# MQinghe/UST-RUN

Hardware: AMD Instinct MI355X
Metric: train images/sec (256x256 U-Net, mixed lb+ulb batch) (higher is better)
Workload: dtype bf16; 1 GPU; fundus 256x256, 2-class U-Net (31.0M params), batch=16+16 per GPU, SSL step = 3 teacher + 5(+1) student forwards, 4 backwards, CE+Dice, SGD+EMA; global_batch=32, parallelism=dp1, fft_mix=device

## Files before the change

### ust-run_amd/csrc/conv_halo_bf16.hip

```cpp
#include "common.h"
#include "loader.h"
#include <stdlib.h>
#include <type_traits>

namespace ustrun {
namespace {

typedef __attribute__((ext_vector_type(8))) elt_t bf16x8;
typedef __attribute__((ext_vector_type(4))) elt_t bf16x4;
typedef __attribute__((address_space(1))) const void gptr_t;
typedef __attribute__((address_space(3))) void lptr_t;


__device__ __attribute__((aligned(16))) const unsigned g_zero16[4] = {0u, 0u, 0u, 0u};

template <int V> using ic = std::integral_constant<int, V>;
template <class T> struct more_value { static constexpr bool value = true; };
template <bool B> struct more_value<std::integral_constant<bool, B>> { static constexpr bool value = B; };

template <int TH, int TW, int BN, int BK, int MI, bool POOL, int NT, bool XF, int DIL = 1, bool BREG = false, bool M16 = false, bool BNS = false,
          int LINW = 0>
__global__ __launch_bounds__(256, (TH * TW * BN >= 512 * 64 && BN == 64 ? 1 : 2)) void conv3x3_halo_bf16_kernel(const IgemmArgs a, const int tiles_x, const int tiles_y,
                                                                   const int nt_total) {
    static_assert(BK == 32, "80-byte patch rows hold one 32-channel chunk");
    constexpr bool LIN = LINW > 0;
    constexpr int RP = LINW + 1;
    constexpr int TM = TH * TW;
    static_assert(!LIN || (DIL == 1 && !POOL && TW == 32 && BREG && RP > 8), "linear tiles: un-dilated, un-pooled, 32-position sub-tiles");
    static_assert(!M16 || (BREG && !XF), "the 16x16x32 build: plain sources, weights through registers");
    static_assert(!BNS || M16, "BatchNorm-backward sums ride on the 16x16x32 epilogue (8 channels of a pixel per lane)");
    static_assert(!BREG || NT <= 2, "register-fed weights: 16 registers per tap and set");
    constexpr int HW2 = LIN ? RP : TW + 2 * DIL;
    constexpr int SR = 32 / TW;
    constexpr int WM = TH / (SR * MI), WN = 4 / WM;
    static_assert(WM * WN == 4 && BN == WN * 64, "4 waves, 64 channels per wave");
    constexpr int HP = LIN ? TM + 2 * RP + 2 : (TH + 2 * DIL) * HW2;
    constexpr int PITCH = 80;
    constexpr int DSLOTS = (HP * 5 + 63) / 64 * 64;
    constexpr int XSLOTS = (HP * 4 + 63) / 64 * 64;
    constexpr int AIT = (DSLOTS + 255) / 256;
    constexpr int NSTG = (9 + NT - 1) / NT;
    constexpr int BATCH = (AIT + NSTG - 2) / (NSTG - 1);
    static_assert(BATCH * (NSTG - 1) >= AIT, "staging fits the chunk");
    constexpr int NP = POOL ? 4 : 1;
    constexpr int ABYTES = (BREG ? AIT * 256 : DSLOTS) * 16;
    constexpr int BCH = (BK / 8) * BN;
    constexpr int BIT = BCH / 256;
    static_assert(BCH % 256 == 0, "B tile must be a whole number of wave-instructions per wave");
    constexpr int RAWB = XF ? BATCH * NP * 4096 : 0;
    constexpr int BBYTES = BREG ? 0 : 2 * NT * BCH * 16;
    constexpr bool SKEW = XF && 2 * ABYTES + BBYTES + 2 * RAWB + 512 <= 81920;
    constexpr int NRAW = SKEW ? 2 : 1;

    extern __shared__ __attribute__((aligned(16))) char smem[];
    char* As = smem;
    char* Bs = smem + 2 * ABYTES;
    char* Raw = Bs + BBYTES;
    char* Cst = Raw + NRAW * RAWB;

    const int IS = LIN ? (a.Ho + 1) * RP : 1;
    const int lin_full = LIN ? a.N / tiles_y : 0;
    const int mt_total = LIN ? lin_full * tiles_x + ((a.N - lin_full * tiles_y) * IS + TM - 1) / TM : a.N * tiles_y * tiles_x;
    const int ntiles = mt_total * nt_total;
    int bid = blockIdx.x;
    {
        const int q = ntiles / 8, r = ntiles % 8, xcd = bid % 8, j = bid / 8;
        bid = (xcd < r ? xcd * (q + 1) : r * (q + 1) + (xcd - r) * q) + j;
    }
    const int mtile = bid / nt_total, ntile = bid % nt_total;
    const int n0 = ntile * BN;
    const int lpass = LIN ? min(mtile / tiles_x, lin_full) : 0;
    const int img = LIN ? lpass * tiles_y : mtile / (tiles_y * tiles_x);
    const int nimg = LIN ? min(tiles_y, a.N - img) : 1;
    const int P0 = LIN ? (mtile - lpass * tiles_x) * TM : 0;
    const int trem = LIN ? 0 : mtile - img * tiles_y * tiles_x;
    const int y0 = LIN ? 0 : (trem / tiles_x) * TH, x0 = LIN ? 0 : (trem % tiles_x) * TW;

    const int tid = threadIdx.x, lane = tid & 63;
    const int wave = __builtin_amdgcn_readfirstlane(tid >> 6);
    const int wm = wave / WN, wn = wave % WN;
    const int l31 = lane & 31, lh = lane >> 5;

    const int nchunk = a.Cin / BK;
    const int K8 = a.Cin / 8;
    const elt_t* Wp = (const elt_t*)a.W;
    const elt_t* zsrc = (const elt_t*)g_zero16;
    const bool wflip = a.dstep < 0;

    constexpr int OOB = (int)0x80000000;
    int aoff[AIT];
    unsigned aokm = 0;
    __amdgpu_buffer_rsrc_t ars = __builtin_amdgcn_make_buffer_rsrc((void*)g_zero16, 0, 0, 0x00020000);
    int asoff = 0;
    int cur_src = -1;
    float a_floor = 0.f;
    const elt_t* aptr = nullptr;
    long dq1 = 0, dq2 = 0;
    f32x4 asc0, asc1, ash0, ash1;
    const int p8 = tid & 3;
    auto src_setup = [&](const SrcDev& S) {
        a_floor = S.relu ? 0.f : -__builtin_inff();
        dq1 = S.sW; dq2 = S.sH;
        const int by = y0 - DIL - S.off_y, bx = x0 - DIL - S.off_x;
        aokm = 0;
        int tq = tid;
        asm volatile("" : "+v"(tq));
#pragma unroll
        for (int i = 0; i < AIT; ++i) {
            const int q = tq + 256 * i;
            const int hp = XF ? (q >> 2) : q / 5;
            const int g = XF ? (tq & 3) : q - 5 * hp;
            if constexpr (LIN) {
                const int F = P0 - RP - 1 + hp, Fc = F < 0 ? 0 : F;
                const int il = Fc / IS, rem = Fc - il * IS, r = rem / RP, c = rem - r * RP;
                const int ly = r - S.off_y, lx = c - S.off_x;
                const bool ok = hp < HP && g < 4 && F >= 0 && il < nimg && r < a.Ho && c < LINW && ly >= 0 && ly < S.LH && lx >= 0 && lx < S.LW;
                aoff[i] = ok ? 2 * ((int)((long)il * S.sN + (long)ly * S.sH + (long)lx * S.sW) + 8 * g) : OOB;
                aokm |= (ok ? 1u : 0u) << i;
                continue;
            }
            const int hy = hp / HW2, hx = hp - hy * HW2;
            const int ly = by + hy, lx = bx + hx;
            const bool ok = hp < HP && g < 4 && ly >= 0 && ly < S.LH && lx >= 0 && lx < S.LW;
            aoff[i] = ok ? 2 * ((int)((POOL ? 2 : 1) * ((long)ly * S.sH + (long)lx * S.sW)) + 8 * g) : OOB;
            aokm |= (ok ? 1u : 0u) << i;
        }
        ars = __builtin_amdgcn_make_buffer_rsrc((void*)((const char*)S.ptr + (long)img * S.sN * 2), 0, 0x7fffffff, 0x00020000);
    };
    auto stage_begin = [&](int c, bool from_lds = true) {
        const int cg = c * BK;
        const int second = (a.nsrc == 2 && cg >= a.src[0].C) ? 1 : 0;
        const SrcDev S = pick_src(a.src[0], a.src[1], second != 0);
        const int cl = cg - (second ? a.src[0].C : 0);
        if (second != cur_src) { src_setup(S); cur_src = second; }
        aptr = (const elt_t*)S.ptr + (img * S.sN + cl);
        asoff = 2 * cl;
        asc0 = asc1 = (f32x4){1.f, 1.f, 1.f, 1.f}; ash0 = ash1 = (f32x4){0.f, 0.f, 0.f, 0.f};
        if (S.scale && !from_lds) {
            const long goff = S.gN > 0 ? (long)(img / S.gN) * S.gstride : 0;
            const float* sc = S.scale + goff + cl + 8 * p8;
            const float* sh = S.shift + goff + cl + 8 * p8;
            asc0 = *(const f32x4*)sc; asc1 = *(const f32x4*)(sc + 4);
            ash0 = *(const f32x4*)sh; ash1 = *(const f32x4*)(sh + 4);
        } else if (S.scale) {
            const char* cs = Cst + (c & 1) * 256 + p8 * 32;
            asc0 = *(const f32x4*)cs; asc1 = *(const f32x4*)(cs + 16);
            ash0 = *(const f32x4*)(cs + 128); ash1 = *(const f32x4*)(cs + 144);
        }
    };
    auto dma_consts = [&](int c) {
        const int cg = c * BK;
        const bool second = (a.nsrc == 2 && cg >= a.src[0].C);
        const SrcDev S = pick_src(a.src[0], a.src[1], second);
        const int cl = cg - (second ? a.src[0].C : 0);
        if (S.scale && wave == 0 && lane < 16) {
            const long goff = S.gN > 0 ? (long)(img / S.gN) * S.gstride : 0;
            const float* src = (lane < 8 ? S.scale : S.shift) + goff + cl + 4 * (lane & 7);
            __builtin_amdgcn_global_load_lds((gptr_t*)src, (lptr_t*)(Cst + (c & 1) * 256), 16, 0, 0);
        }
// ... 4 lines not shown
        if constexpr (XF) {
#pragma unroll
            for (int q = 0; q < NP; ++q) {
                const int d = 2 * (int)((q & 1 ? dq1 : 0) + (q & 2 ? dq2 : 0));
                dma16_buf_s(vo, ars, asoff + d, raw + ((b * NP + q) * 256 + wave * 64) * 16);
            }
        } else {
            dma16_buf_s(vo, ars, asoff, Adst + (256 * i + wave * 64) * 16);
        }
    };
    auto act8 = [&](bf16x8 r, f32x4& lo, f32x4& hi) {
        lo = (f32x4){(float)r[0], (float)r[1], (float)r[2], (float)r[3]} * asc0 + ash0;
        hi = (f32x4){(float)r[4], (float)r[5], (float)r[6], (float)r[7]} * asc1 + ash1;
#pragma unroll
        for (int q = 0; q < 4; ++q) {
            lo[q] = __builtin_amdgcn_fmed3f(lo[q], a_floor, __builtin_inff());
            hi[q] = __builtin_amdgcn_fmed3f(hi[q], a_floor, __builtin_inff());
        }
    };
    typedef __attribute__((ext_vector_type(4))) unsigned u32x4;
    auto xform8 = [&](const bf16x8* r, bool inimg) {
        f32x4 lo, hi;
        act8(r[0], lo, hi);
#pragma unroll
        for (int q = 1; q < NP; ++q) {
            f32x4 l2, h2;
            act8(r[q], l2, h2);
            lo = max4(lo, l2); hi = max4(hi, h2);
        }
        bf16x8 h;
        h[0] = (elt_t)lo[0]; h[1] = (elt_t)lo[1]; h[2] = (elt_t)lo[2]; h[3] = (elt_t)lo[3];
        h[4] = (elt_t)hi[0]; h[5] = (elt_t)hi[1]; h[6] = (elt_t)hi[2]; h[7] = (elt_t)hi[3];
        u32x4 u = __builtin_bit_cast(u32x4, h);
#pragma unroll
        for (int q = 0; q < 4; ++q) u[q] = inimg ? u[q] : 0u;
        return __builtin_bit_cast(bf16x8, u);
    };
    const int xw0 = (tid >> 2) * PITCH + p8 * 16;
    auto raw_read = [&](int b, const char* raw, bf16x8* r) {
#pragma unroll
        for (int q = 0; q < NP; ++q) r[q] = *(const bf16x8*)(raw + ((b * NP + q) * 256 + tid) * 16);
    };
    auto xform_store = [&](int i, const bf16x8* r, char* Adst, bool live, const char* raw) {
        const bool in_patch = live && (tid >> 2) + 64 * i < HP;
        char* dst = in_patch ? Adst + xw0 + i * 64 * PITCH : (char*)raw + tid * 16;
        *(bf16x8*)dst = xform8(r, (aokm >> i) & 1u);
    };
    const elt_t* wthr[BIT];
#pragma unroll
    for (int i = 0; i < BIT; ++i) {
        const int idx = tid + 256 * i, o = idx / BN, n = idx % BN;
        wthr[i] = Wp + ((long)o * a.Cout + n0 + n) * 8;
    }
    auto dma_B = [&](int c, int tap, int slot) {
        const int wt = wflip ? 8 - tap : tap;
        const long woff = ((long)wt * K8 + c * (BK / 8)) * a.Cout * 8;
        char* dst = Bs + slot * (BCH * 16);
#pragma unroll
        for (int i = 0; i < BIT; ++i)
            __builtin_amdgcn_global_load_lds((gptr_t*)(wthr[i] + woff), (lptr_t*)(dst + (wave * 64 + 256 * i) * 16), 16, 0, 0);
    };

    const __amdgpu_buffer_rsrc_t wrs = __builtin_amdgcn_make_buffer_rsrc((void*)Wp, 0, (int)min((long)9 * K8 * a.Cout * 16, 0x7fffffffL), 0x00020000);
    const int bvoff0 = (lh * a.Cout + n0 + wn * 64 + l31) * 16, bvoff1 = bvoff0 + 2 * a.Cout * 16;
    const int bvoff16 = ((lane >> 4) * a.Cout + n0 + wn * 64 + (lane & 15)) * 16;
    bf16x8 bnx[NT][BK / 16][2];
    auto load_B = [&](int c, int tap, int k) {
        const int wt = wflip ? 8 - tap : tap;
        const int soff = __builtin_amdgcn_readfirstlane((int)(((long)wt * K8 + c * (BK / 8)) * a.Cout * 16));
        if constexpr (M16)
            asm volatile("s_nop 4\n\tbuffer_load_dwordx4 %0, %4, %5, %6 offen\n\tbuffer_load_dwordx4 %1, %4, %5, %6 offen offset:256\n\t"
                         "buffer_load_dwordx4 %2, %4, %5, %6 offen offset:512\n\tbuffer_load_dwordx4 %3, %4, %5, %6 offen offset:768"
                         : "=&v"(bnx[k][0][0]), "=&v"(bnx[k][0][1]), "=&v"(bnx[k][1][0]), "=&v"(bnx[k][1][1])
                         : "v"(bvoff16), "s"(wrs), "s"(soff) : "memory");
        else
        asm volatile("s_nop 4\n\tbuffer_load_dwordx4 %0, %4, %6, %7 offen\n\tbuffer_load_dwordx4 %1, %4, %6, %7 offen offset:512\n\t"
                     "buffer_load_dwordx4 %2, %5, %6, %7 offen\n\tbuffer_load_dwordx4 %3, %5, %6, %7 offen offset:512"
                     : "=&v"(bnx[k][0][0]), "=&v"(bnx[k][0][1]), "=&v"(bnx[k][1][0]), "=&v"(bnx[k][1][1])
                     : "v"(bvoff0), "v"(bvoff1), "s"(wrs), "s"(soff) : "memory");
    };

    f32x16 acc[M16 ? 1 : MI][2];
    f32x4 acc16[M16 ? MI : 1][2][4];
#pragma unroll
    for (int i = 0; i < (M16 ? 1 : MI); ++i)
#pragma unroll
        for (int j = 0; j < 2; ++j)
#pragma unroll
            for (int r = 0; r < 16; ++r) acc[i][j][r] = 0.f;
#pragma unroll
    for (int i = 0; i < (M16 ? MI : 1); ++i)
#pragma unroll
        for (int h = 0; h < 2; ++h)
#pragma unroll
            for (int g = 0; g < 4; ++g) acc16[i][h][g] = (f32x4){0.f, 0.f, 0.f, 0.f};

    const int afrag0 = LIN ? (M16 ? (wm * MI * 32 + (lane & 15)) * PITCH + (lane >> 4) * 16 : (wm * MI * 32 + l31) * PITCH + lh * 16)
                     : M16 ? ((wm * SR * MI) * HW2 + (lane & 15)) * PITCH + (lane >> 4) * 16
                           : ((wm * SR * MI + (TW == 16 ? (l31 >> 4) : 0)) * HW2 + (l31 & (TW - 1))) * PITCH + lh * 16;
    const int bfrag0 = (lh * BN + wn * 64 + l31) * 16;
    const int nstage = nchunk * NSTG;

    if constexpr (BREG) {
#pragma unroll
        for (int k = 0; k < NT; ++k) load_B(0, k, k);
    } else {
#pragma unroll
        for (int k = 0; k < NT; ++k) dma_B(0, k, k);
    }
    if (nchunk > 1) dma_consts(1);
    stage_begin(0, false);
    if constexpr (XF) {
        bf16x8 pv[AIT][NP];
#pragma unroll
        for (int i = 0; i < AIT; ++i) {
            const bool ok = (aokm >> i) & 1u;
            const elt_t* src = ok ? (const elt_t*)((const char*)aptr + aoff[i]) : zsrc;
#pragma unroll
            for (int q = 0; q < NP; ++q) pv[i][q] = *(const bf16x8*)(src + (ok ? (q & 1 ? dq1 : 0) + (q & 2 ? dq2 : 0) : 0));
        }
#pragma unroll
        for (int i = 0; i < AIT; ++i)
        {
            const bool in_patch = (tid >> 2) + 64 * i < HP;
            *(bf16x8*)(in_patch ? As + xw0 + i * 64 * PITCH : Raw + tid * 16) = xform8(pv[i], (aokm >> i) & 1u);
        }
    } else {
#pragma unroll
        for (int i = 0; i < AIT; ++i)
            if (wave_has(i)) issue_one(i, 0, As, nullptr);
    }
    asm volatile("s_waitcnt vmcnt(0)" ::: "memory");
    __syncthreads();

    bf16x8 acar[MI];
    constexpr bool PEEL = BREG && !XF;
    constexpr bool CT = BREG && XF && SKEW;
    constexpr bool APIPE = BREG && !XF;
    int ni_prev = 0;
    auto chunk = [&](const int c, auto more_c) __attribute__((always_inline)) {
        const bool more = more_c;
        constexpr bool morec = more_value<decltype(more_c)>::value;
        const char* Afrag = As + (c & 1) * ABYTES + afrag0;
        char* Anext = As + ((c + 1) & 1) * ABYTES;
        if (more) stage_begin(c + 1);
        auto stage = [&](auto ic_j) {
            constexpr int j = decltype(ic_j)::value;
            constexpr int t0 = j * NT, nt = (9 - t0 < NT) ? 9 - t0 : NT;
            constexpr int jn = (j + 1) % NSTG, tn0 = jn * NT, nn = (9 - tn0 < NT) ? 9 - tn0 : NT;
            const int s = c * NSTG + j;
            bf16x8 bcur[NT][BK / 16][2];
            const bool has_next = PEEL ? (morec || j < NSTG - 1) : (CT || s + 1 < nstage);
            const int nb_new = (BREG && has_next) ? 4 * nn : 0;
            if constexpr (BREG) {
#pragma unroll
                for (int k = 0; k < NT; ++k)
#pragma unroll
                    for (int ks = 0; ks < BK / 16; ++ks) { bcur[k][ks][0] = bnx[k][ks][0]; bcur[k][ks][1] = bnx[k][ks][1]; }
                if (has_next) {
#pragma unroll
                    for (int k = 0; k < nn; ++k) load_B(jn == 0 ? (CT && !more ? c : c + 1) : c, tn0 + k, k);
                }
            } else if (s + 1 < nstage) {
#pragma unroll
                for (int k = 0; k < nn; ++k) dma_B(jn == 0 ? c + 1 : c, tn0 + k, ((s + 1) & 1) * NT + k);
            }
            if constexpr (j == NSTG - 1) { if (c + 2 < nchunk) dma_consts(c + 2); }
            char* rawW = Raw + (SKEW ? (s & 1) * RAWB : 0);
            const char* rawR = Raw + (SKEW ? ((s & 1) ^ 1) * RAWB : 0);
            int ni = 0;
            if constexpr (j < NSTG - 1) {
                if (CT || more) {
#pragma unroll
                    for (int b = 0; b < BATCH; ++b) {
                        constexpr int dummy = 0; (void)dummy;
                        if (j * BATCH + b < AIT && wave_has(j * BATCH + b)) { issue_one(j * BATCH + b, b, Anext, rawW, more); ni += NP; }
                    }
                }
            }
            __builtin_amdgcn_sched_barrier(0);
            if constexpr (BREG) {
                if constexpr (PEEL || CT) {
                    constexpr auto pieces = [](int jj) constexpr {
                        int n = 0;
                        if ((CT || morec) && jj >= 0 && jj < NSTG - 1)
                            for (int b = 0; b < BATCH; ++b) n += (jj * BATCH + b < AIT) ? NP : 0;
                        return n;
                    };
                    constexpr int younger = ((CT || morec || j < NSTG - 1) ? 4 * nn : 0) + pieces(j) + (XF ? 0 : pieces(j - 1));
                    static_assert(younger < 64, "vmcnt is a 6-bit counter");
                    asm volatile("s_waitcnt vmcnt(%0)" :: "n"(younger) : "memory");
                } else {
                    const int younger = nb_new + ni + (XF ? 0 : ni_prev);
                    switch (younger < 12 ? younger : 12) {
                        case 12: asm volatile("s_waitcnt vmcnt(12)" ::: "memory"); break;
                        case 11: asm volatile("s_waitcnt vmcnt(11)" ::: "memory"); break;
                        case 10: asm volatile("s_waitcnt vmcnt(10)" ::: "memory"); break;
                        case 9: asm volatile("s_waitcnt vmcnt(9)" ::: "memory"); break;
                        case 8: asm volatile("s_waitcnt vmcnt(8)" ::: "memory"); break;
                        case 7: asm volatile("s_waitcnt vmcnt(7)" ::: "memory"); break;
                        case 6: asm volatile("s_waitcnt vmcnt(6)" ::: "memory"); break;
                        case 5: asm volatile("s_waitcnt vmcnt(5)" ::: "memory"); break;
                        case 4: asm volatile("s_waitcnt vmcnt(4)" ::: "memory"); break;
                        case 3: asm volatile("s_waitcnt vmcnt(3)" ::: "memory"); break;
                        case 2: asm volatile("s_waitcnt vmcnt(2)" ::: "memory"); break;
                        case 1: asm volatile("s_waitcnt vmcnt(1)" ::: "memory"); break;
                        default: asm volatile("s_waitcnt vmcnt(0)" ::: "memory"); break;
                    }
                    ni_prev = ni;
                }
#pragma unroll
                for (int k = 0; k < NT; ++k)
#pragma unroll
                    for (int ks = 0; ks < BK / 16; ++ks) asm volatile("" : "+v"(bcur[k][ks][0]), "+v"(bcur[k][ks][1]));
                __builtin_amdgcn_sched_barrier(0);
            }
            auto afrag = [&](int tap, int ks, int i) __attribute__((always_inline)) {
                if constexpr (LIN)
                    return *(const bf16x8*)(Afrag + (32 * i + (M16 ? 16 * ks : 0) + (tap / 3) * RP + tap % 3) * PITCH + (M16 ? 0 : ks * 32));
                else if constexpr (M16)
                    return *(const bf16x8*)(Afrag + ((DIL * (tap / 3) + SR * i + (TW == 16 ? ks : 0)) * HW2 + DIL * (tap % 3) + (TW == 16 ? 0 : 16 * ks)) * PITCH);
                else
                return *(const bf16x8*)(Afrag + ((DIL * (tap / 3) + SR * i) * HW2 + DIL * (tap % 3)) * PITCH + ks * 32);
            };
            if constexpr (APIPE) {
                if constexpr (j == 0) {
#pragma unroll
// ... 89 lines not shown
                            for (int g = 0; g < 4; ++g)
                                acc16[i][ks][g] = USTRUN_MFMA_16x16x32(bf[k][g >> 1][g & 1], af[k][ks][i], acc16[i][ks][g], 0, 0, 0);
                        } else {
                        acc[i][0] = USTRUN_MFMA_32x32x16(af[k][ks][i], bf[k][ks][0], acc[i][0], 0, 0, 0);
                        acc[i][1] = USTRUN_MFMA_32x32x16(af[k][ks][i], bf[k][ks][1], acc[i][1], 0, 0, 0);
                        }
                    }
            }
            if constexpr (SKEW) {
#pragma unroll
                for (int b = 0; b < nitem; ++b) xform_store(jx * BATCH + b, rr[b], Anext, more, rawR);
            }
            constexpr int nmfma = nt * (BK / 16) * MI * (M16 ? 4 : 2);
            constexpr int vpm = !SKEW ? 0 : (nitem * (NP * 26 + 14) + nmfma - 1) / nmfma;
            if constexpr (APIPE) {
                if constexpr ((j == 0 ? MI : 0) + nitem * NP > 0) __builtin_amdgcn_sched_group_barrier(0x100, (j == 0 ? MI : 0) + nitem * NP, 0);
                if constexpr (M16) {
#pragma unroll
                    for (int h = 0; h < nt * (BK / 16); ++h) {
                        const bool next_read = h + 1 < nt * (BK / 16) || j < NSTG - 1;
#pragma unroll
                        for (int i = 0; i < MI; ++i) {
                            __builtin_amdgcn_sched_group_barrier(0x008, 4, 0);
                            if (next_read) __builtin_amdgcn_sched_group_barrier(0x100, 1, 0);
                        }
                    }
                } else
#pragma unroll
                for (int h = 0; h < nt * (BK / 16); ++h) {
                    const bool next_read = h + 1 < nt * (BK / 16) || j < NSTG - 1;
#pragma unroll
                    for (int m = 0; m < (M16 ? 4 : 2) * MI; ++m) {
                        if (m == 2 && next_read) __builtin_amdgcn_sched_group_barrier(0x100, MI, 0);
                        __builtin_amdgcn_sched_group_barrier(0x008, 1, 0);
                        if constexpr (vpm > 0) __builtin_amdgcn_sched_group_barrier(0x002, vpm, 0);
                    }
                }
                if constexpr (nitem > 0) __builtin_amdgcn_sched_group_barrier(0x200, nitem, 0);
            } else if constexpr (SKEW) {
                constexpr int nread = nt * (BK / 16) * ((BREG ? 0 : 2) + MI) + nitem * NP;
                __builtin_amdgcn_sched_group_barrier(0x100, nread, 0);
#pragma unroll
                for (int m = 0; m < nmfma; ++m) {
                    __builtin_amdgcn_sched_group_barrier(0x008, 1, 0);
                    if constexpr (vpm > 0) __builtin_amdgcn_sched_group_barrier(0x002, vpm, 0);
                }
                if constexpr (nitem > 0) __builtin_amdgcn_sched_group_barrier(0x200, nitem, 0);
            }
            __builtin_amdgcn_sched_barrier(0);
            if constexpr (BREG && j < NSTG - 1 && (!XF || SKEW)) {
            } else if constexpr (!XF && j < NSTG - 1) {
                if (ni == 0) asm volatile("s_waitcnt vmcnt(0)" ::: "memory");
                else if (ni == 1) asm volatile("s_waitcnt vmcnt(1)" ::: "memory");
                else asm volatile("s_waitcnt vmcnt(2)" ::: "memory");
            } else {
                asm volatile("s_waitcnt vmcnt(0)" ::: "memory");
            }
            if constexpr (!SKEW && nitem > 0) {
                if (more) {
#pragma unroll
                    for (int b = 0; b < nitem; ++b) {
                        if (256 * (jx * BATCH + b) + wave * 64 < XSLOTS) {
                            raw_read(b, rawR, rr[b]);
                            xform_store(jx * BATCH + b, rr[b], Anext, true, rawR);
                        }
                    }
                }
            }
            if constexpr (!BREG || j == NSTG - 1) {
                asm volatile("s_waitcnt lgkmcnt(0)" ::: "memory");
                __builtin_amdgcn_s_barrier();
            }
            asm volatile("" ::: "memory");
        };
        stage(ic<0>{}); stage(ic<1>{}); stage(ic<2>{}); stage(ic<3>{}); stage(ic<4>{});
        if constexpr (NSTG > 5) { stage(ic<5>{}); stage(ic<6>{}); stage(ic<7>{}); stage(ic<8>{}); }
    };
    if constexpr (PEEL) {
        for (int c = 0; c + 1 < nchunk; ++c) chunk(c, std::true_type{});
        chunk(nchunk - 1, std::false_type{});
    } else {
        for (int c = 0; c < nchunk; ++c) chunk(c, c + 1 < nchunk);
    }

    const int C1 = a.Cout - a.C0;
    typedef __attribute__((ext_vector_type(2))) float f32x2;
    typedef __attribute__((ext_vector_type(2))) elt_t bf16x2;
    f32x2 s1v[2] = {{0.f, 0.f}, {0.f, 0.f}}, s2v[2] = {{0.f, 0.f}, {0.f, 0.f}};
    float s1p[8] = {0.f, 0.f, 0.f, 0.f, 0.f, 0.f, 0.f, 0.f}, s2p[8] = {0.f, 0.f, 0.f, 0.f, 0.f, 0.f, 0.f, 0.f};
    auto stat_piece = [&](const bf16x8 v8, bool ok) {
#pragma unroll
        for (int q = 0; q < 8; ++q) {
            const float f = ok ? (float)v8[q] : 0.f;
            s1p[q] += f; s2p[q] += f * f;
        }
    };
    float bsc[8], bsh[8];
    if constexpr (BNS) {
        const long go = a.bn_gN > 0 ? (long)(img / a.bn_gN) * a.bn_gstride : 0;
        const float* ps = a.bnsc + go + n0 + wn * 64 + (lane & 7) * 8;
        const float* pb = a.bnsh + go + n0 + wn * 64 + (lane & 7) * 8;
        const f32x4 s0 = *(const f32x4*)ps, s1_ = *(const f32x4*)(ps + 4), b0 = *(const f32x4*)pb, b1 = *(const f32x4*)(pb + 4);
#pragma unroll
        for (int q = 0; q < 4; ++q) { bsc[q] = s0[q]; bsc[4 + q] = s1_[q]; bsh[q] = b0[q]; bsh[4 + q] = b1[q]; }
    }
    auto bns_piece = [&](const bf16x8 v8, const bf16x8 y8, bool ok) {
#pragma unroll
        for (int q = 0; q < 8; ++q) {
            const float yf = (float)y8[q];
            const float dz = (ok && yf * bsc[q] + bsh[q] > 0.f) ? (float)v8[q] : 0.f;
            s1p[q] += dz; s2p[q] += dz * yf;
        }
    };
    constexpr int EPITCH = 144;
    char* ep = smem + wave * (32 * EPITCH);
    const bool full = !LIN && y0 + TH <= a.Ho && x0 + TW <= a.Wo;
    int e_il = 0, e_r = 0, e_c = 0;
    unsigned vmask = 0xffffffffu;
    auto lin_pos = [&](int P, int& il, int& r, int& c) { il = P / IS; const int rem = P - il * IS; r = rem / RP; c = rem - r * RP; };
    if constexpr (LIN) lin_pos(P0 + wm * MI * 32 + (lane >> 3), e_il, e_r, e_c);
    auto park = [&](int i, auto mask_c, auto stat_c) {
        constexpr bool MASK = decltype(mask_c)::value, STAT = decltype(stat_c)::value;
        const int oyb = y0 + wm * SR * MI + SR * i;
        if constexpr (M16) {
#pragma unroll
            for (int h = 0; h < 2; ++h)
#pragma unroll
                for (int g = 0; g < 4; ++g) {
                    const f32x4 v = acc16[M16 ? i : 0][h][g];
                    bf16x4 h4;
                    h4[0] = (elt_t)v[0]; h4[1] = (elt_t)v[1]; h4[2] = (elt_t)v[2]; h4[3] = (elt_t)v[3];
                    *(bf16x4*)(ep + (16 * h + (lane & 15)) * EPITCH + (16 * g + 4 * (lane >> 4)) * 2) = h4;
                }
        } else {
#pragma unroll
        for (int j = 0; j < 2; ++j) {
#pragma unroll
            for (int r = 0; r < 16; r += 2) {
                const int row = (r & 3) + 8 * (r >> 2) + 4 * lh;
                const f32x2 v = {acc[M16 ? 0 : i][j][r], acc[M16 ? 0 : i][j][r + 1]};
                const bf16x2 h = __builtin_convertvector(v, bf16x2);
                *(elt_t*)(ep + row * EPITCH + (j * 32 + l31) * 2) = h[0];
                *(elt_t*)(ep + (row + 1) * EPITCH + (j * 32 + l31) * 2) = h[1];
                if (!STAT) continue;
                f32x2 f = __builtin_convertvector(h, f32x2);
                if (MASK && LIN) {
                    if (!((vmask >> row) & 1u)) f[0] = 0.f;
                    if (!((vmask >> (row + 1)) & 1u)) f[1] = 0.f;
                } else if (MASK) {
                    const int oy0 = oyb + (TW == 16 ? (row >> 4) : 0), ox0 = x0 + (row & (TW - 1));
                    const int oy1 = oyb + (TW == 16 ? ((row + 1) >> 4) : 0), ox1 = x0 + ((row + 1) & (TW - 1));
                    if (!(oy0 < a.Ho && ox0 < a.Wo)) f[0] = 0.f;
                    if (!(oy1 < a.Ho && ox1 < a.Wo)) f[1] = 0.f;
                }
                s1v[j] += f;
                s2v[j] += f * f;
            }
        }
        }
    };
#pragma unroll
    for (int i = 0; i < MI; ++i) {
        const int oyb = y0 + wm * SR * MI + SR * i;
        if constexpr (LIN && !M16) {
            if (a.stat) {
                int il, r, c;
                lin_pos(P0 + wm * MI * 32 + 32 * i + l31, il, r, c);
                vmask = (unsigned)__builtin_amdgcn_ballot_w64(il < nimg && r < a.Ho && c < LINW);
            }
        }
        if constexpr (M16) park(i, std::false_type{}, std::false_type{});
        else {
        if (!a.stat) park(i, std::false_type{}, std::false_type{});
        else if (full) park(i, std::false_type{}, std::true_type{});
        else park(i, std::true_type{}, std::true_type{});
        }
        __builtin_amdgcn_fence(__ATOMIC_RELEASE, "wavefront");
        __builtin_amdgcn_wave_barrier();
        __builtin_amdgcn_fence(__ATOMIC_ACQUIRE, "wavefront");
        if (full && n0 + wn * 64 + 64 <= a.C0) {
            const int r0 = lane >> 3, ch = lane & 7;
            elt_t* base = (elt_t*)a.out0 + (((long)img * a.Ho + oyb) * a.Wo + x0) * a.C0 + n0 + wn * 64 + ch * 8;
#pragma unroll
            for (int t = 0; t < 4; ++t) {
                const int row = r0 + 8 * t;
                const bf16x8 v8 = *(const bf16x8*)(ep + row * EPITCH + ch * 16);
                const long off = TW == 16 ? ((long)(row >> 4) * a.Wo + (row & 15)) * a.C0 : (long)row * a.C0;
                *(bf16x8*)(base + off) = v8;
                if constexpr (BNS) bns_piece(v8, *(const bf16x8*)((const elt_t*)a.bny + (base - (elt_t*)a.out0) + off), true);
                else if constexpr (M16) { if (a.stat) stat_piece(v8, true); }
            }
        } else
#pragma unroll
        for (int t = 0; t < 4; ++t) {
            const int idx = lane + 64 * t, row = idx >> 3, ch = idx & 7;
            const bf16x8 v8 = *(const bf16x8*)(ep + row * EPITCH + ch * 16);
            const int oy = LIN ? e_r : oyb + (TW == 16 ? (row >> 4) : 0), ox = LIN ? e_c : x0 + (row & (TW - 1));
            const int oimg = LIN ? img + e_il : img;
            const bool inb = LIN ? (e_il < nimg && e_r < a.Ho && e_c < LINW) : (oy < a.Ho && ox < a.Wo);
            if constexpr (LIN) {
                e_c += 8;
                if (e_c >= RP) { e_c -= RP; if (++e_r > a.Ho) { e_r = 0; ++e_il; } }
            }
            const int col = n0 + wn * 64 + ch * 8;
            if constexpr (BNS) {
                const bool ok = inb && col < a.C0;
                const long eo = ok ? (((long)oimg * a.Ho + oy) * a.Wo + ox) * a.C0 + col : 0;
                bns_piece(v8, *(const bf16x8*)((const elt_t*)a.bny + eo), ok);
            } else if constexpr (M16) { if (a.stat) stat_piece(v8, inb); }
            if (inb) {
                if (col < a.C0) {
                    *(bf16x8*)((elt_t*)a.out0 + (((long)oimg * a.Ho + oy) * a.Wo + ox) * a.C0 + col) = v8;
                } else {
                    const int y1 = oy - a.o1y, x1 = ox - a.o1x;
                    if (y1 >= 0 && y1 < a.H1 && x1 >= 0 && x1 < a.W1)
                        *(bf16x8*)((elt_t*)a.out1 + (((long)oimg * a.H1 + y1) * a.W1 + x1) * C1 + (col - a.C0)) = v8;
                }
            }
        }
        __builtin_amdgcn_fence(__ATOMIC_RELEASE, "wavefront");
        __builtin_amdgcn_wave_barrier();
        __builtin_amdgcn_fence(__ATOMIC_ACQUIRE, "wavefront");
    }
    float s1[2] = {s1v[0][0] + s1v[0][1], s1v[1][0] + s1v[1][1]}, s2[2] = {s2v[0][0] + s2v[0][1], s2v[1][0] + s2v[1][1]};
    if (a.stat) {
        float* red = (float*)(smem + 4 * 32 * EPITCH);
        if constexpr (M16) {
#pragma unroll
            for (int q = 0; q < 8; ++q) {
#pragma unroll
                for (int o = 8; o < 64; o <<= 1) { s1p[q] += __shfl_xor(s1p[q], o); s2p[q] += __shfl_xor(s2p[q], o); }
                if (lane < 8) {
                    red[(wm * 2 + 0) * BN + wn * 64 + lane * 8 + q] = s1p[q];
                    red[(wm * 2 + 1) * BN + wn * 64 + lane * 8 + q] = s2p[q];
                }
            }
        } else
#pragma unroll
        for (int j = 0; j < 2; ++j) {
            s1[j] += __shfl_xor(s1[j], 32);
            s2[j] += __shfl_xor(s2[j], 32);
            if (lh == 0) {
                red[(wm * 2 + 0) * BN + wn * 64 + j * 32 + l31] = s1[j];
                red[(wm * 2 + 1) * BN + wn * 64 + j * 32 + l31] = s2[j];
            }
        }
        __syncthreads();
        constexpr int SROWS = TH / 8;
        constexpr int WPS = WM / SROWS;
        for (int t = tid; t < SROWS * 2 * BN; t += 256) {
            const int h = t / (2 * BN), q = (t / BN) % 2, cc = t % BN;
            float v = 0.f;
#pragma unroll
            for (int w = 0; w < WPS; ++w) v += red[((h * WPS + w) * 2 + q) * BN + cc];
            a.stat[((long)(mtile * SROWS + h) * 2 + q) * a.Cout + n0 + cc] = v;
        }
    }
}

thread_local int g_last_variant = 0;

struct LinPlan { int gN, tpp, mtiles, last_rows; };
static LinPlan lin_plan(const IgemmArgs& a) {
    int g = a.pass_gN > 0 ? a.pass_gN : 0;
    for (int i = 0; i < a.nsrc && !g; ++i)
        if (a.src[i].gN > 0) g = a.src[i].gN;
    if (!g && a.bn_gN > 0) g = a.bn_gN;
    if (g <= 0 || g > a.N) g = a.N;
    const long IS = (long)(a.Ho + 1) * (a.Wo + 1);
    const int tpp = (int)cdiv(g * IS, 256L), full = a.N / g, tailN = a.N - full * g, tail = (int)cdiv(tailN * IS, 256L);
    return {g, tpp, full * tpp + tail, tailN ? tail : (full > 1 ? tpp : -1)};
}

template <int TH, int TW, int BN, int BK, int MI, bool POOL, int NT, bool XF, int DIL = 1, bool BREG = false, bool M16 = false, bool BNS = false,
          int LINW = 0>
int launch_xf(const IgemmArgs& a, hipStream_t st) {
    g_last_variant = (LINW ? (1 << 30 | LINW << 16) : (TH << 24 | TW << 16)) | BN << 8 | (M16 ? 0x80 : 0) | MI << 4 | NT << 2 | (POOL ? 2 : 0) | (XF ? 1 : 0);
    const LinPlan lp = LINW ? lin_plan(a) : LinPlan{0, 0, 0, -1};
    const int tx = LINW ? lp.tpp : cdiv(a.Wb, TW), ty = LINW ? lp.gN : cdiv(a.Hb, TH), nt = a.Cout / BN;
    constexpr int DSLOTS = ((LINW ? TH * TW + 2 * (LINW + 1) + 2 : (TH + 2 * DIL) * (TW + 2 * DIL)) * 5 + 63) / 64 * 64;
    constexpr int AIT = (DSLOTS + 255) / 256, NSTG = (9 + NT - 1) / NT, BATCH = (AIT + NSTG - 2) / (NSTG - 1);
    const size_t rawb = XF ? (size_t)BATCH * (POOL ? 4 : 1) * 4096 : 0;
    const size_t fixed = 2 * (size_t)(BREG ? AIT * 256 : DSLOTS) * 16 + (BREG ? 0 : 2 * NT * (size_t)(BK / 8) * BN * 16) + 512;
    const size_t lds = fixed + (XF && fixed + 2 * rawb <= 81920 ? 2 : 1) * rawb;
    dim3 grid((LINW ? lp.mtiles : a.N * ty * tx) * nt), block(256);
    if (lds > 64 * 1024)
        USTRUN_TRY(ensure_dynamic_lds((const void*)conv3x3_halo_bf16_kernel<TH, TW, BN, BK, MI, POOL, NT, XF, DIL, BREG, M16, BNS, LINW>, (int)lds, "conv3x3_halo_bf16"));
    hipLaunchKernelGGL((conv3x3_halo_bf16_kernel<TH, TW, BN, BK, MI, POOL, NT, XF, DIL, BREG, M16, BNS, LINW>), grid, block, lds, st, a, tx, ty, nt);
    USTRUN_LAUNCH_CHECK("conv3x3_halo_bf16");
    return 0;
}

template <int TH, int TW, int BN, int BK, int MI, bool POOL, int NT = 1>
int launch_cfg(const IgemmArgs& a, hipStream_t st) {
    bool xf = POOL;
    for (int i = 0; i < a.nsrc; ++i) xf |= a.src[i].scale != nullptr || a.src[i].relu != 0;
    if constexpr (POOL) return launch_xf<TH, TW, BN, BK, MI, POOL, NT, true>(a, st);
    else {
        {
            {
                const bool m16 = !(g_debug_flags & 8) && !(g_debug_flags & 2097152) && ((g_debug_flags & 32768) || (!xf && MI == 4 && NT == 1));
                if constexpr (MI == 4 && NT == 1 && BN == 128) {
                    if (a.bny) {
                        USTRUN_CHECK(m16 && !xf && a.stat && a.bnsc && a.bnsh, "conv3x3_halo: BatchNorm-backward sums need a plain source on the 16x16x32 build");
                        return launch_xf<TH, TW, BN, BK, MI, POOL, NT, false, 1, true, true, true>(a, st);
                    }
                }
                if (m16 && !xf)
                    return launch_xf<TH, TW, BN, BK, MI, POOL, NT, false, 1, true, true>(a, st);
            }
            if (!(g_debug_flags & 8))
                return xf ? launch_xf<TH, TW, BN, BK, MI, POOL, NT, true, 1, true>(a, st) : launch_xf<TH, TW, BN, BK, MI, POOL, NT, false, 1, true>(a, st);
        }
        return xf ? launch_xf<TH, TW, BN, BK, MI, POOL, NT, true>(a, st) : launch_xf<TH, TW, BN, BK, MI, POOL, NT, false>(a, st);
    }
}

}

int halo_last_variant() { return g_last_variant; }
static int halo_dilation(const IgemmArgs& a) { return a.dstep < 0 ? -a.dstep : a.dstep; }
void set_last_variant(int v) { g_last_variant = v; }

int halo_stat_rows(int N, int H, int W) { return N * cdiv(H, 8) * cdiv(W, 16); }

bool halo_supported(const IgemmArgs& a) {
    if (a.nseg != 9 || a.nz != 1 || a.s_in != 1 || a.s_out != 1 || a.segw != 3) return false;
    const int dil = a.dstep < 0 ? -a.dstep : a.dstep;
    if (a.d0 != -a.dstep || !(dil == 1 || dil == 2 || dil == 4)) return false;
    bool pool = false;
    if (a.out_esz != 2 || (a.C0 & 7) || ((a.Cout - a.C0) & 7) || a.bias) return false;
    for (int i = 0; i < a.nsrc; ++i) {
        if (a.src[i].sC != 1 || (a.src[i].C & 7) || a.src[i].esz != 2) return false;
        pool |= a.src[i].pool != 0;
    }
    const int BK = 32;
    if (a.Cin % BK || a.Cout % 64) return false;
    if (a.nsrc == 2 && (a.src[0].C % BK)) return false;
    if (pool && (a.nsrc != 1 || a.Cout % 128)) return false;
    if (a.Hb < 4 || a.Wb < 8) return false;
    if (dil > 1 && (pool || a.nsrc != 1)) return false;
    return true;
}

int halo_tile128(const IgemmArgs& a);
static double halo_rect_score(const IgemmArgs& a);

int halo_linear_w(const IgemmArgs& a) {
    if ((g_debug_flags2 & 1) || (g_debug_flags & (8 | 2097152 | 32768)) || ((g_debug_flags >> 10) & 3)) return 0;
    if (!halo_supported(a) || halo_dilation(a) != 1 || a.Cout % 128 || a.Hb != a.Ho || a.Wb != a.Wo) return 0;
    const int w = a.Wo;
    if (!(w == 18 || w == 24 || w == 36 || w == 72)) return 0;
    int g = a.pass_gN > 0 ? a.pass_gN : 0;
    for (int i = 0; i < a.nsrc; ++i) {
        if (a.src[i].pool) return 0;
        if (a.src[i].gN > 0) { if (g && g != a.src[i].gN) return 0; g = a.src[i].gN; }
    }
    if (a.bny && a.bn_gN > 0 && g && g != a.bn_gN) return 0;
    const LinPlan lp = lin_plan(a);
    for (int i = 0; i < a.nsrc; ++i)
        if ((long)lp.gN * a.src[i].sN * 2 >= (1L << 31) - 4096) return 0;
    if ((long)lp.mtiles * (a.Cout / 128) < 160) return 0;
    const double lin = (double)a.N * a.Ho * a.Wo / (lp.mtiles * 256.0);
    return lin > 1.05 * halo_rect_score(a) ? w : 0;
}
int halo_linear_last_pass_rows(const IgemmArgs& a) { return halo_linear_w(a) ? lin_plan(a).last_rows : -1; }

bool halo_bnsum_supported(const IgemmArgs& a) {
    if (!halo_supported(a) || a.nsrc != 1 || a.out1 || a.C0 != a.Cout || a.Cout % 128) return false;
    if (a.src[0].scale || a.src[0].relu || a.src[0].pool) return false;
    if ((g_debug_flags & (8 | 2097152))) return false;
// ... 112 lines not shown
```

Baseline: 1161 images/sec.

## Add persistent walking mode to 8x32 halo conv that chains tiles per block

For the plain-source 8x32 M16 halo conv variant, launches a reduced grid (about 512/nt blocks, sized per group) in which each block walks a contiguous run of spatial tiles. The next tile's prologue (weight and patch loads) is issued into the alternate patch buffer before the current tile's epilogue, and the epilogue scratch is moved into the finished buffer. This aims to cut block launch and prologue latency and overlap the next tile's loads with the store epilogue. In exchange it adds more complex buffer-parity bookkeeping and possible load imbalance from the fixed partitioning.

```diff
diff --git a/ust-run_amd/csrc/conv_halo_bf16.hip b/ust-run_amd/csrc/conv_halo_bf16.hip
--- a/ust-run_amd/csrc/conv_halo_bf16.hip
+++ b/ust-run_amd/csrc/conv_halo_bf16.hip
@@ -18,11 +18,13 @@
 template <class T> struct more_value { static constexpr bool value = true; };
 template <bool B> struct more_value<std::integral_constant<bool, B>> { static constexpr bool value = B; };
 
+struct WalkPlan { int g, bfull, btail, run; };
 template <int TH, int TW, int BN, int BK, int MI, bool POOL, int NT, bool XF, int DIL = 1, bool BREG = false, bool M16 = false, bool BNS = false,
-          int LINW = 0>
+          int LINW = 0, bool WALK = false>
 __global__ __launch_bounds__(256, (TH * TW * BN >= 512 * 64 && BN == 64 ? 1 : 2)) void conv3x3_halo_bf16_kernel(const IgemmArgs a, const int tiles_x, const int tiles_y,
-                                                                   const int nt_total) {
+                                                                   const int nt_total, const WalkPlan wp) {
     static_assert(BK == 32, "80-byte patch rows hold one 32-channel chunk");
+    static_assert(!WALK || (LINW == 0 && BREG && !XF && !BNS && !POOL && DIL == 1 && TH == 8 && TW == 32), "walking form: the 8 x 32 tiles, plain sources, register-fed weights");
     constexpr bool LIN = LINW > 0;
     constexpr int RP = LINW + 1;
     constexpr int TM = TH * TW;
@@ -64,17 +66,29 @@
     const int ntiles = mt_total * nt_total;
     int bid = blockIdx.x;
     {
-        const int q = ntiles / 8, r = ntiles % 8, xcd = bid % 8, j = bid / 8;
+        const int nb = WALK ? (int)gridDim.x : ntiles;
+        const int q = nb / 8, r = nb % 8, xcd = bid % 8, j = bid / 8;
         bid = (xcd < r ? xcd * (q + 1) : r * (q + 1) + (xcd - r) * q) + j;
     }
-    const int mtile = bid / nt_total, ntile = bid % nt_total;
+    int mtile = bid / nt_total;
+    const int ntile = bid % nt_total;
+    int tend = 0;
+    if constexpr (WALK) {
+        const int tpi = tiles_y * tiles_x, nfull = a.N / wp.g;
+        const int p = min(mtile / wp.bfull, nfull), pb = mtile - p * wp.bfull;
+        const int T = (p < nfull ? wp.g : a.N - nfull * wp.g) * tpi, B = p < nfull ? wp.bfull : wp.btail;
+        const int f = wp.run ? pb * wp.run : (int)((long)pb * T / B);
+        const int l = wp.run ? min(f + wp.run, T) : (int)((long)(pb + 1) * T / B);
+        mtile = p * wp.g * tpi + f;
+        tend = p * wp.g * tpi + l;
+    }
     const int n0 = ntile * BN;
     const int lpass = LIN ? min(mtile / tiles_x, lin_full) : 0;
-    const int img = LIN ? lpass * tiles_y : mtile / (tiles_y * tiles_x);
+    int img = LIN ? lpass * tiles_y : mtile / (tiles_y * tiles_x);
     const int nimg = LIN ? min(tiles_y, a.N - img) : 1;
     const int P0 = LIN ? (mtile - lpass * tiles_x) * TM : 0;
     const int trem = LIN ? 0 : mtile - img * tiles_y * tiles_x;
-    const int y0 = LIN ? 0 : (trem / tiles_x) * TH, x0 = LIN ? 0 : (trem % tiles_x) * TW;
+    int y0 = LIN ? 0 : (trem / tiles_x) * TH, x0 = LIN ? 0 : (trem % tiles_x) * TW;
 
     const int tid = threadIdx.x, lane = tid & 63;
     const int wave = __builtin_amdgcn_readfirstlane(tid >> 6);
@@ -245,18 +259,21 @@
 
     f32x16 acc[M16 ? 1 : MI][2];
     f32x4 acc16[M16 ? MI : 1][2][4];
-#pragma unroll
-    for (int i = 0; i < (M16 ? 1 : MI); ++i)
-#pragma unroll
-        for (int j = 0; j < 2; ++j)
-#pragma unroll
-            for (int r = 0; r < 16; ++r) acc[i][j][r] = 0.f;
-#pragma unroll
-    for (int i = 0; i < (M16 ? MI : 1); ++i)
-#pragma unroll
-        for (int h = 0; h < 2; ++h)
-#pragma unroll
-            for (int g = 0; g < 4; ++g) acc16[i][h][g] = (f32x4){0.f, 0.f, 0.f, 0.f};
+    auto acc_zero = [&]() {
+#pragma unroll
+        for (int i = 0; i < (M16 ? 1 : MI); ++i)
+#pragma unroll
+            for (int j = 0; j < 2; ++j)
+#pragma unroll
+                for (int r = 0; r < 16; ++r) acc[i][j][r] = 0.f;
+#pragma unroll
+        for (int i = 0; i < (M16 ? MI : 1); ++i)
+#pragma unroll
+            for (int h = 0; h < 2; ++h)
+#pragma unroll
+                for (int g = 0; g < 4; ++g) acc16[i][h][g] = (f32x4){0.f, 0.f, 0.f, 0.f};
+    };
+    if constexpr (!WALK) acc_zero();
 
     const int afrag0 = LIN ? (M16 ? (wm * MI * 32 + (lane & 15)) * PITCH + (lane >> 4) * 16 : (wm * MI * 32 + l31) * PITCH + lh * 16)
                      : M16 ? ((wm * SR * MI) * HW2 + (lane & 15)) * PITCH + (lane >> 4) * 16
@@ -264,37 +281,45 @@
     const int bfrag0 = (lh * BN + wn * 64 + l31) * 16;
     const int nstage = nchunk * NSTG;
 
-    if constexpr (BREG) {
-#pragma unroll
-        for (int k = 0; k < NT; ++k) load_B(0, k, k);
-    } else {
-#pragma unroll
-        for (int k = 0; k < NT; ++k) dma_B(0, k, k);
-    }
-    if (nchunk > 1) dma_consts(1);
-    stage_begin(0, false);
-    if constexpr (XF) {
-        bf16x8 pv[AIT][NP];
-#pragma unroll
-        for (int i = 0; i < AIT; ++i) {
-            const bool ok = (aokm >> i) & 1u;
-            const elt_t* src = ok ? (const elt_t*)((const char*)aptr + aoff[i]) : zsrc;
-#pragma unroll
-            for (int q = 0; q < NP; ++q) pv[i][q] = *(const bf16x8*)(src + (ok ? (q & 1 ? dq1 : 0) + (q & 2 ? dq2 : 0) : 0));
-        }
-#pragma unroll
-        for (int i = 0; i < AIT; ++i)
-        {
-            const bool in_patch = (tid >> 2) + 64 * i < HP;
-            *(bf16x8*)(in_patch ? As + xw0 + i * 64 * PITCH : Raw + tid * 16) = xform8(pv[i], (aokm >> i) & 1u);
-        }
-    } else {
-#pragma unroll
-        for (int i = 0; i < AIT; ++i)
-            if (wave_has(i)) issue_one(i, 0, As, nullptr);
-    }
+    int pbase = 0;
+    auto prologue = [&]() {
+        char* A0 = As + pbase * ABYTES;
+        if constexpr (BREG) {
+#pragma unroll
+            for (int k = 0; k < NT; ++k) load_B(0, k, k);
+        } else {
+#pragma unroll
+            for (int k = 0; k < NT; ++k) dma_B(0, k, k);
+        }
+        if constexpr (!WALK) { if (nchunk > 1) dma_consts(1); }
+        else cur_src = -1;
+        stage_begin(0, false);
+        if constexpr (XF) {
+            bf16x8 pv[AIT][NP];
+#pragma unroll
+            for (int i = 0; i < AIT; ++i) {
+                const bool ok = (aokm >> i) & 1u;
+                const elt_t* src = ok ? (const elt_t*)((const char*)aptr + aoff[i]) : zsrc;
+#pragma unroll
+                for (int q = 0; q < NP; ++q) pv[i][q] = *(const bf16x8*)(src + (ok ? (q & 1 ? dq1 : 0) + (q & 2 ? dq2 : 0) : 0));
+            }
+#pragma unroll
+            for (int i = 0; i < AIT; ++i)
+            {
+                const bool in_patch = (tid >> 2) + 64 * i < HP;
+                *(bf16x8*)(in_patch ? A0 + xw0 + i * 64 * PITCH : Raw + tid * 16) = xform8(pv[i], (aokm >> i) & 1u);
+            }
+        } else {
+#pragma unroll
+            for (int i = 0; i < AIT; ++i)
+                if (wave_has(i)) issue_one(i, 0, A0, nullptr);
+        }
+    };
+    prologue();
+    for (;;) {
     asm volatile("s_waitcnt vmcnt(0)" ::: "memory");
     __syncthreads();
+    if constexpr (WALK) acc_zero();
 
     bf16x8 acar[MI];
     constexpr bool PEEL = BREG && !XF;
@@ -304,8 +329,8 @@
     auto chunk = [&](const int c, auto more_c) __attribute__((always_inline)) {
         const bool more = more_c;
         constexpr bool morec = more_value<decltype(more_c)>::value;
-        const char* Afrag = As + (c & 1) * ABYTES + afrag0;
-        char* Anext = As + ((c + 1) & 1) * ABYTES;
+        const char* Afrag = As + ((c + pbase) & 1) * ABYTES + afrag0;
+        char* Anext = As + ((c + 1 + pbase) & 1) * ABYTES;
         if (more) stage_begin(c + 1);
         auto stage = [&](auto ic_j) {
             constexpr int j = decltype(ic_j)::value;
@@ -561,7 +586,25 @@
     } else {
         for (int c = 0; c < nchunk; ++c) chunk(c, c + 1 < nchunk);
     }
-
+    const int emt = mtile, eimg = img, ey0 = y0, ex0 = x0;
+    const int ebuf = WALK ? (nchunk - 1 + pbase) & 1 : 0;
+    bool walk_on = false;
+    if constexpr (WALK) {
+        walk_on = ++mtile < tend;
+        if (walk_on) {
+            const int tpi = tiles_y * tiles_x;
+            img = mtile / tpi;
+            const int tr = mtile - img * tpi;
+            y0 = (tr / tiles_x) * TH; x0 = (tr % tiles_x) * TW;
+            pbase = ebuf ^ 1;
+            prologue();
+        }
+    }
+
+    int tid_e = tid;
+    if constexpr (WALK) asm volatile("" : "+v"(tid_e));
+    {
+    const int tid = tid_e, lane = tid & 63, l31 = lane & 31, lh = lane >> 5;
     const int C1 = a.Cout - a.C0;
     typedef __attribute__((ext_vector_type(2))) float f32x2;
     typedef __attribute__((ext_vector_type(2))) elt_t bf16x2;
@@ -576,7 +619,7 @@
     };
     float bsc[8], bsh[8];
     if constexpr (BNS) {
-        const long go = a.bn_gN > 0 ? (long)(img / a.bn_gN) * a.bn_gstride : 0;
+        const long go = a.bn_gN > 0 ? (long)(eimg / a.bn_gN) * a.bn_gstride : 0;
         const float* ps = a.bnsc + go + n0 + wn * 64 + (lane & 7) * 8;
         const float* pb = a.bnsh + go + n0 + wn * 64 + (lane & 7) * 8;
         const f32x4 s0 = *(const f32x4*)ps, s1_ = *(const f32x4*)(ps + 4), b0 = *(const f32x4*)pb, b1 = *(const f32x4*)(pb + 4);
@@ -592,15 +635,16 @@
         }
     };
     constexpr int EPITCH = 144;
-    char* ep = smem + wave * (32 * EPITCH);
-    const bool full = !LIN && y0 + TH <= a.Ho && x0 + TW <= a.Wo;
+    static_assert(!WALK || 4 * 32 * EPITCH + WM * 2 * BN * 4 <= ABYTES, "the epilogue's scratch fits one patch buffer");
+    char* ep = smem + ebuf * ABYTES + wave * (32 * EPITCH);
+    const bool full = !LIN && ey0 + TH <= a.Ho && ex0 + TW <= a.Wo;
     int e_il = 0, e_r = 0, e_c = 0;
     unsigned vmask = 0xffffffffu;
     auto lin_pos = [&](int P, int& il, int& r, int& c) { il = P / IS; const int rem = P - il * IS; r = rem / RP; c = rem - r * RP; };
     if constexpr (LIN) lin_pos(P0 + wm * MI * 32 + (lane >> 3), e_il, e_r, e_c);
     auto park = [&](int i, auto mask_c, auto stat_c) {
         constexpr bool MASK = decltype(mask_c)::value, STAT = decltype(stat_c)::value;
-        const int oyb = y0 + wm * SR * MI + SR * i;
+        const int oyb = ey0 + wm * SR * MI + SR * i;
         if constexpr (M16) {
 #pragma unroll
             for (int h = 0; h < 2; ++h)
@@ -627,8 +671,8 @@
                     if (!((vmask >> row) & 1u)) f[0] = 0.f;
                     if (!((vmask >> (row + 1)) & 1u)) f[1] = 0.f;
                 } else if (MASK) {
-                    const int oy0 = oyb + (TW == 16 ? (row >> 4) : 0), ox0 = x0 + (row & (TW - 1));
-                    const int oy1 = oyb + (TW == 16 ? ((row + 1) >> 4) : 0), ox1 = x0 + ((row + 1) & (TW - 1));
+                    const int oy0 = oyb + (TW == 16 ? (row >> 4) : 0), ox0 = ex0 + (row & (TW - 1));
+                    const int oy1 = oyb + (TW == 16 ? ((row + 1) >> 4) : 0), ox1 = ex0 + ((row + 1) & (TW - 1));
                     if (!(oy0 < a.Ho && ox0 < a.Wo)) f[0] = 0.f;
                     if (!(oy1 < a.Ho && ox1 < a.Wo)) f[1] = 0.f;
                 }
@@ -640,7 +684,7 @@
     };
 #pragma unroll
     for (int i = 0; i < MI; ++i) {
-        const int oyb = y0 + wm * SR * MI + SR * i;
+        const int oyb = ey0 + wm * SR * MI + SR * i;
         if constexpr (LIN && !M16) {
             if (a.stat) {
                 int il, r, c;
@@ -659,7 +703,7 @@
         __builtin_amdgcn_fence(__ATOMIC_ACQUIRE, "wavefront");
         if (full && n0 + wn * 64 + 64 <= a.C0) {
             const int r0 = lane >> 3, ch = lane & 7;
-            elt_t* base = (elt_t*)a.out0 + (((long)img * a.Ho + oyb) * a.Wo + x0) * a.C0 + n0 + wn * 64 + ch * 8;
+            elt_t* base = (elt_t*)a.out0 + (((long)eimg * a.Ho + oyb) * a.Wo + ex0) * a.C0 + n0 + wn * 64 + ch * 8;
 #pragma unroll
             for (int t = 0; t < 4; ++t) {
                 const int row = r0 + 8 * t;
@@ -674,8 +718,8 @@
         for (int t = 0; t < 4; ++t) {
             const int idx = lane + 64 * t, row = idx >> 3, ch = idx & 7;
             const bf16x8 v8 = *(const bf16x8*)(ep + row * EPITCH + ch * 16);
-            const int oy = LIN ? e_r : oyb + (TW == 16 ? (row >> 4) : 0), ox = LIN ? e_c : x0 + (row & (TW - 1));
-            const int oimg = LIN ? img + e_il : img;
+            const int oy = LIN ? e_r : oyb + (TW == 16 ? (row >> 4) : 0), ox = LIN ? e_c : ex0 + (row & (TW - 1));
+            const int oimg = LIN ? eimg + e_il : eimg;
             const bool inb = LIN ? (e_il < nimg && e_r < a.Ho && e_c < LINW) : (oy < a.Ho && ox < a.Wo);
             if constexpr (LIN) {
                 e_c += 8;
@@ -703,7 +747,7 @@
     }
     float s1[2] = {s1v[0][0] + s1v[0][1], s1v[1][0] + s1v[1][1]}, s2[2] = {s2v[0][0] + s2v[0][1], s2v[1][0] + s2v[1][1]};
     if (a.stat) {
-        float* red = (float*)(smem + 4 * 32 * EPITCH);
+        float* red = (float*)(smem + ebuf * ABYTES + 4 * 32 * EPITCH);
         if constexpr (M16) {
 #pragma unroll
             for (int q = 0; q < 8; ++q) {
@@ -732,8 +776,11 @@
             float v = 0.f;
 #pragma unroll
             for (int w = 0; w < WPS; ++w) v += red[((h * WPS + w) * 2 + q) * BN + cc];
-            a.stat[((long)(mtile * SROWS + h) * 2 + q) * a.Cout + n0 + cc] = v;
-        }
+            a.stat[((long)(emt * SROWS + h) * 2 + q) * a.Cout + n0 + cc] = v;
+        }
+    }
+    }
+    if (!walk_on) break;
     }
 }
 
@@ -749,6 +796,26 @@
     const long IS = (long)(a.Ho + 1) * (a.Wo + 1);
     const int tpp = (int)cdiv(g * IS, 256L), full = a.N / g, tailN = a.N - full * g, tail = (int)cdiv(tailN * IS, 256L);
     return {g, tpp, full * tpp + tail, tailN ? tail : (full > 1 ? tpp : -1)};
+}
+
+static bool walk_plan(const IgemmArgs& a, int tpi, int nt, WalkPlan& wp) {
+    if (g_debug_flags2 & 16) return false;
+    int g = a.pass_gN > 0 ? a.pass_gN : 0;
+    for (int i = 0; i < a.nsrc; ++i)
+        if (a.src[i].gN > 0) { if (g && g != a.src[i].gN) return false; g = a.src[i].gN; }
+    if (g <= 0 || g > a.N) g = a.N;
+    const int nfull = a.N / g, tailN = a.N - nfull * g;
+    const long Tf = (long)g * tpi, Tt = (long)tailN * tpi;
+    if (Tf * (nfull + 1) >= (1L << 30)) return false;
+    if (g_debug_flags2 & 32) {
+        wp = {g, (int)cdiv(Tf, 3L), (int)cdiv(Tt, 3L), 3};
+        return true;
+    }
+    const int slots = 512 / nt;
+    const int bfull = (int)((long)slots * g / a.N), btail = (int)((long)slots * tailN / a.N);
+    if (bfull < 1 || Tf / bfull < 4 || (tailN && (btail < 1 || Tt / btail < 4))) return false;
+    wp = {g, bfull, btail, 0};
+    return true;
 }
 
 template <int TH, int TW, int BN, int BK, int MI, bool POOL, int NT, bool XF, int DIL = 1, bool BREG = false, bool M16 = false, bool BNS = false,
@@ -763,9 +830,24 @@
     const size_t fixed = 2 * (size_t)(BREG ? AIT * 256 : DSLOTS) * 16 + (BREG ? 0 : 2 * NT * (size_t)(BK / 8) * BN * 16) + 512;
     const size_t lds = fixed + (XF && fixed + 2 * rawb <= 81920 ? 2 : 1) * rawb;
     dim3 grid((LINW ? lp.mtiles : a.N * ty * tx) * nt), block(256);
+    constexpr bool WALKABLE = TH == 8 && TW == 32 && DIL == 1 && LINW == 0 && BREG && !BNS && !POOL && !XF &&
+                              BN == 128 && MI == 4 && NT == 1 && M16;
+    if constexpr (WALKABLE) {
+        WalkPlan wp;
+        if (walk_plan(a, ty * tx, nt, wp)) {
+            g_last_variant |= 0x800;
+            const int nfull = a.N / wp.g;
+            dim3 wgrid((nfull * wp.bfull + (a.N > nfull * wp.g ? wp.btail : 0)) * nt);
+            if (lds > 64 * 1024)
+                USTRUN_TRY(ensure_dynamic_lds((const void*)conv3x3_halo_bf16_kernel<TH, TW, BN, BK, MI, POOL, NT, XF, DIL, BREG, M16, BNS, LINW, true>, (int)lds, "conv3x3_halo_bf16"));
+            hipLaunchKernelGGL((conv3x3_halo_bf16_kernel<TH, TW, BN, BK, MI, POOL, NT, XF, DIL, BREG, M16, BNS, LINW, true>), wgrid, block, lds, st, a, tx, ty, nt, wp);
+            USTRUN_LAUNCH_CHECK("conv3x3_halo_bf16");
+            return 0;
+        }
+    }
     if (lds > 64 * 1024)
         USTRUN_TRY(ensure_dynamic_lds((const void*)conv3x3_halo_bf16_kernel<TH, TW, BN, BK, MI, POOL, NT, XF, DIL, BREG, M16, BNS, LINW>, (int)lds, "conv3x3_halo_bf16"));
-    hipLaunchKernelGGL((conv3x3_halo_bf16_kernel<TH, TW, BN, BK, MI, POOL, NT, XF, DIL, BREG, M16, BNS, LINW>), grid, block, lds, st, a, tx, ty, nt);
+    hipLaunchKernelGGL((conv3x3_halo_bf16_kernel<TH, TW, BN, BK, MI, POOL, NT, XF, DIL, BREG, M16, BNS, LINW>), grid, block, lds, st, a, tx, ty, nt, WalkPlan{0, 0, 0, 0});
     USTRUN_LAUNCH_CHECK("conv3x3_halo_bf16");
     return 0;
 }
```

Result: slower. 1146 images/sec (-1.3%).
